# alexlee-gk/video_prediction

Measured on AMD Instinct MI355X. Metric: train frames/sec (whole node), BAIR 64x64 seq30 SAVP, higher is better.
Workload: dtype bf16

## Files before the change

video_prediction_amd/csrc/common.hip:

```cpp
#include <hip/hip_runtime.h>
#include <dlfcn.h>
#include <string.h>
#include "savp_hip.h"
#include "opts.h"
#include "conv_common.h"

extern "C" const char* savp_version(void) { return "savp_hip 0.1 gfx950"; }

thread_local hipEvent_t g_savp_prof_start = nullptr;
thread_local hipEvent_t g_savp_prof_stop = nullptr;

extern "C" int savp_prof_event_create(void** ev) {
    if (!ev) return SAVP_EINVAL;
    hipEvent_t e;
    if (hipEventCreate(&e) != hipSuccess) return SAVP_ELAUNCH;
    *ev = (void*)e;
    return SAVP_OK;
}
extern "C" int savp_prof_event_destroy(void* ev) { return (ev && hipEventDestroy((hipEvent_t)ev) == hipSuccess) ? SAVP_OK : SAVP_EINVAL; }
extern "C" int savp_prof_arm(void* start, void* stop) {
    if ((start == nullptr) != (stop == nullptr)) return SAVP_EINVAL;
    g_savp_prof_start = (hipEvent_t)start; g_savp_prof_stop = (hipEvent_t)stop;
    return SAVP_OK;
}
extern "C" int savp_prof_armed(void) { return g_savp_prof_start != nullptr; }
extern "C" int savp_prof_elapsed_us(void* start, void* stop, float* us) {
    if (!start || !stop || !us) return SAVP_EINVAL;
    float ms = 0.f;
    if (hipEventElapsedTime(&ms, (hipEvent_t)start, (hipEvent_t)stop) != hipSuccess) return SAVP_ELAUNCH;
    *us = ms * 1e3f;
    return SAVP_OK;
}

static struct { const char* name; int value; } g_opts[OPT_COUNT] = {
    {"conv_ring", 0}, {"s2dgrad", 1}, {"thin", 1}, {"wgp_cfg", 0}, {"wgp_split", 0}, {"inorm_min_hw", 64}, {"colsum_2stage", 1},
    {"dense_legacy", 0}, {"cdna_legacy", 0}, {"lstm_fused", 1}, {"ring_dma", 1}, {"lstm_q", 0}, {"ring_wwarm", 1}, {"wgp_dma", 1}, {"ring_early", 1}, {"gate_kernel", 1}, {"gate_alt", 0}, {"gate_cell", 1}, {"gate_wwarm", 1}, {"inorm_fast", 1}, {"inorm_fast_taken", 0}, {"splitk_reduced", 0}, {"ring_fixed", 1}, {"ring_fixed_taken", 0}, {"fd_fixed", 1}, {"fd_fixed_taken", 0},
};
int savp_opt(int id) { return g_opts[id].value; }
void savp_opt_count(int id) { ++g_opts[id].value; }
extern "C" int savp_set_option(const char* name, int value) {
    if (!name) return SAVP_EINVAL;
    for (int i = 0; i < OPT_COUNT; ++i)
        if (!strcmp(g_opts[i].name, name)) { g_opts[i].value = value; return SAVP_OK; }
    return SAVP_EINVAL;
}
extern "C" int savp_get_option(const char* name, int* value) {
    if (!name || !value) return SAVP_EINVAL;
    for (int i = 0; i < OPT_COUNT; ++i)
        if (!strcmp(g_opts[i].name, name)) { *value = g_opts[i].value; return SAVP_OK; }
    return SAVP_EINVAL;
}

typedef int (*rccl_allreduce_fn)(const void*, void*, size_t, int, int, void*, hipStream_t);
extern "C" int savp_allreduce_bucket(void* comm, void* stream, void* buf, int64_t count) {
    if (!comm || !buf || count < 0) return SAVP_EINVAL;
    if (count == 0) return SAVP_OK;
    static rccl_allreduce_fn fn = nullptr;
    if (!fn) {
        void* h = dlopen("librccl.so", RTLD_NOW | RTLD_GLOBAL);
        if (!h) h = dlopen("librccl.so.1", RTLD_NOW | RTLD_GLOBAL);
        if (!h) h = dlopen("/opt/rocm/lib/librccl.so", RTLD_NOW | RTLD_GLOBAL);
        if (!h) return SAVP_ELAUNCH;
        fn = (rccl_allreduce_fn)dlsym(h, "ncclAllReduce");
        if (!fn) return SAVP_ELAUNCH;
    }
    return fn(buf, buf, (size_t)count, 7, 0, comm, (hipStream_t)stream) == 0 ? SAVP_OK : SAVP_ELAUNCH;
}

int splitk_fit(const SavpConvArgs* a, int want, long long block_elems) {
    if (want <= 1) return 1;
    if (!a->ws || a->ws_bytes <= 0 || block_elems <= 0 || (((uintptr_t)a->ws) & 15)) { savp_opt_count(OPT_SPLITK_REDUCED); return 1; }
    const long long fit = a->ws_bytes / (block_elems * (long long)sizeof(float));
    if (fit < want) savp_opt_count(OPT_SPLITK_REDUCED);
    if (fit < 2) return 1;
    return want < fit ? want : (int)fit;
}

__global__ __launch_bounds__(256) void splitk_fold_kernel(float* __restrict__ out, const float* __restrict__ part, int splitk, long long n4, long long n,
                                                          int beta, int Cd, int gap_at, int gap) {
    const long long stride = (long long)gridDim.x * 256;
    for (long long i = (long long)blockIdx.x * 256 + threadIdx.x; i < n4; i += stride) {
        float4 s = beta ? reinterpret_cast<const float4*>(out)[i] : make_float4(0.f, 0.f, 0.f, 0.f);
        for (int k = 0; k < splitk; ++k) {
            const float4 v = reinterpret_cast<const float4*>(part + (long long)k * n)[i];
            s.x += v.x; s.y += v.y; s.z += v.z; s.w += v.w;
        }
        if (gap) {
            const int c = (int)((i * 4) % Cd);
            float* e = &s.x;
#pragma unroll
            for (int j = 0; j < 4; ++j)
                if (c + j >= gap_at && c + j < gap_at + gap) e[j] = beta ? reinterpret_cast<const float*>(out)[i * 4 + j] : 0.f;
        }
        reinterpret_cast<float4*>(out)[i] = s;
    }
}

__global__ __launch_bounds__(256) void splitk_fold_scalar_kernel(float* __restrict__ out, const float* __restrict__ part, int splitk, long long n, int beta,
                                                                 int Cd, int gap_at, int gap) {
    const long long stride = (long long)gridDim.x * 256;
    for (long long i = (long long)blockIdx.x * 256 + threadIdx.x; i < n; i += stride) {
        const int c = (int)(i % Cd);
        if (gap && c >= gap_at && c < gap_at + gap) { if (!beta) out[i] = 0.f; continue; }
        float s = beta ? out[i] : 0.f;
        for (int k = 0; k < splitk; ++k) s += part[(long long)k * n + i];
        out[i] = s;
    }
}

void splitk_fold(float* out, const float* part, int splitk, long long n, int beta, int Cd, int gap_at, int gap, hipStream_t st) {
    const bool vec = (n % 4 == 0) && (Cd % 4 == 0) && ((((uintptr_t)out) & 15) == 0) && ((((uintptr_t)part) & 15) == 0);
    const long long work = vec ? n / 4 : n;
    long long blocks = (work + 255) / 256;
    if (blocks > 2048) blocks = 2048;
    if (blocks < 1) blocks = 1;
    if (vec) hipLaunchKernelGGL(splitk_fold_kernel, dim3((unsigned)blocks), dim3(256), 0, st, out, part, splitk, n / 4, n, beta, Cd, gap_at, gap);
    else hipLaunchKernelGGL(splitk_fold_scalar_kernel, dim3((unsigned)blocks), dim3(256), 0, st, out, part, splitk, n, beta, Cd, gap_at, gap);
}

typedef float fold_f4 __attribute__((ext_vector_type(4)));
template <bool VEC>
__global__ __launch_bounds__(256) void wgrad_fold_kernel(float* __restrict__ out, const float* __restrict__ part, int nsplit, long long n, long long slice) {
    const long long i = (long long)blockIdx.x * 256 + threadIdx.x;
    if (i >= n) return;
    if constexpr (VEC) {
        fold_f4 s = reinterpret_cast<const fold_f4*>(out)[i];
        const fold_f4* __restrict__ q = reinterpret_cast<const fold_f4*>(part) + i;
        const long long st4 = slice >> 2;
        int k = 0;
        for (; k + 8 <= nsplit; k += 8) {
            fold_f4 v[8];
#pragma unroll
            for (int j = 0; j < 8; ++j) v[j] = __builtin_nontemporal_load(q + (long long)(k + j) * st4);
#pragma unroll
            for (int j = 0; j < 8; ++j) s += v[j];
        }
        for (; k < nsplit; ++k) s += __builtin_nontemporal_load(q + (long long)k * st4);
        reinterpret_cast<fold_f4*>(out)[i] = s;
    } else {
        float s = out[i];
        for (int k = 0; k < nsplit; ++k) s += part[(long long)k * slice + i];
        out[i] = s;
    }
}

void wgrad_fold(float* out, const float* part, int nsplit, long long n, hipStream_t st, long long slice) {
    if (nsplit < 1 || n <= 0) return;
    if (slice <= 0) slice = n;
    const bool vec = (n % 4 == 0) && (slice % 4 == 0) && ((((uintptr_t)out) & 15) == 0) && ((((uintptr_t)part) & 15) == 0);
    const long long work = vec ? n / 4 : n;
    const unsigned blocks = (unsigned)((work + 255) / 256);
    if (vec) hipLaunchKernelGGL(wgrad_fold_kernel<true>, dim3(blocks), dim3(256), 0, st, out, part, nsplit, work, slice);
    else hipLaunchKernelGGL(wgrad_fold_kernel<false>, dim3(blocks), dim3(256), 0, st, out, part, nsplit, work, slice);
}
```

video_prediction_amd/csrc/conv_gate.hip:

```cpp
#include "conv_common.h"
#include "opts.h"
#include <hip/hip_ext.h>
#include <type_traits>

extern thread_local hipEvent_t g_savp_prof_start;
extern thread_local hipEvent_t g_savp_prof_stop;

struct GateP {
    const unsigned short* x;
    const uint4* wfrag;
    unsigned short* y;
    double* stats;
    const void* zero16;
    int N, Cy, mtiles, ntiles;
    int wwarm;
    int F; float eps, forget_bias;
    const float* c_prev; long long cp_sn, cp_sp;
    const float *g1, *b1, *g2, *b2;
    float* c_new;
    int nh; void* h[4]; long long h_sn[4], h_sp[4]; int h16;
    float *mean1, *rstd1, *mean2, *rstd2;
};

__device__ __attribute__((aligned(16))) unsigned g_gate_zero[4] = {0u, 0u, 0u, 0u};

#ifdef SAVP_GATE_STAMPS
__device__ unsigned long long g_gate_t[4][8];
__constant__ int g_gate_blk = 0;
#define GT(i) do { if ((int)blockIdx.x == g_gate_blk && (threadIdx.x & 63) == 0) g_gate_t[threadIdx.x >> 6][i] = __builtin_readcyclecounter(); } while (0)
extern "C" int savp_debug_gate_times(unsigned long long* out) { return hipMemcpyFromSymbol(out, HIP_SYMBOL(g_gate_t), sizeof(g_gate_t)) == hipSuccess ? 0 : -1; }
extern "C" int savp_debug_gate_block(int b) { return hipMemcpyToSymbol(HIP_SYMBOL(g_gate_blk), &b, sizeof(int)) == hipSuccess ? 0 : -1; }
#else
#define GT(i) do {} while (0)
#endif

__device__ __forceinline__ void gate_touch4(const void* gsrc, unsigned lds_dst) {
    unsigned keep;
    asm volatile("s_mov_b32 %0, m0\n\ts_mov_b32 m0, %2\n\ts_nop 0\n\tglobal_load_lds_dword %1, off\n\ts_mov_b32 m0, %0"
                 : "=&s"(keep) : "v"(gsrc), "s"(lds_dst) : "memory");
}

__device__ __forceinline__ void gate_dma16(const void* gsrc, unsigned lds_dst) {
    unsigned keep;
    asm volatile("s_mov_b32 %0, m0\n\ts_mov_b32 m0, %2\n\ts_nop 0\n\tglobal_load_lds_dwordx4 %1, off\n\ts_mov_b32 m0, %0"
                 : "=&s"(keep) : "v"(gsrc), "s"(lds_dst) : "memory");
}

template <int S, int CIN, int TM, int TN, int NWN>
struct GateCfg {
    static constexpr int KH = 5, KW = 5, PAD = 2, TAPS = KH * KW;
    static constexpr int KSPLIT = 4 / NWN;
    static constexpr int PIX = 32 * TM;
    static constexpr int C8 = CIN / 8;
    static constexpr int C8P = (C8 & 1) ? C8 : C8 + 1;
    static constexpr int PXB = C8P * 16;
    static constexpr int TC = S >= 16 ? 16 : 8;
    static constexpr int TR = (S * S >= PIX) ? PIX / TC : S;
    static constexpr int NI = PIX / (TR * TC);
    static constexpr int PR = TR + 2 * PAD, PC = TC + 2 * PAD;
    static constexpr int RPAD = (256 - (4 * PXB) % 256) % 256;
    static constexpr int RP = PC * PXB + RPAD;
    static constexpr int IMGB = PR * RP;
    static constexpr int PATCHB = NI * IMGB;
    static constexpr int NCH = TAPS * C8;
    static constexpr int KS = (NCH + 1) / 2;
    static constexpr int KPAD = 8;
    static constexpr int ETABB = ((2 * (KS + KPAD) * 4) + 15) & ~15;
    static constexpr int NCW = 32 * TN;
    static constexpr int NC = NCW * NWN;
    static constexpr int TILEB = 32 * 32 * 4;
    static constexpr int XB = (KSPLIT > 1 ? TM / 2 : 0) * TN * TILEB;
    static constexpr int TP = NC / 2 + 4;
    static constexpr int STGB = PIX * TP * 4;
    static constexpr int STATB = KSPLIT * NC * 2 * 4;
    static constexpr int EPIB = (4 * XB > STGB ? 4 * XB : STGB) + STATB;
    static constexpr int WARMB = 256;
    static constexpr int LDSB = (PATCHB + ETABB + WARMB) > EPIB ? (PATCHB + ETABB + WARMB) : EPIB;
    static constexpr int TPI = NI == 1 ? (S / TR) * (S / TC) : 1;
    static constexpr int PPR = PC * C8P;
    static constexpr int NJ = (PPR + 63) / 64;
    static constexpr int aoff(int i) { return ((i * 32) / (TR * TC)) * IMGB + (((i * 32) % (TR * TC)) / TC) * RP; }
    static_assert(CIN % 8 == 0 && S % TC == 0 && S % TR == 0 && (TM == 4 || TM == 8) && (TN == 1 || TN == 2) && (NWN == 1 || NWN == 2) && TR * TC * NI == PIX && 32 % TC == 0, "shape");
    static_assert(LDSB <= 160 * 1024, "LDS");
};

template <int TM, int TN, int I>
__device__ __forceinline__ void gate_sched() {
    constexpr int M = TM * TN, ND = TM + 1, NV = TN;
    if constexpr (I < M) {
        constexpr int d = (ND * (I + 1)) / M - (ND * I) / M;
        constexpr int v = (NV * (I + 1)) / M - (NV * I) / M;
        if constexpr (d > 0) __builtin_amdgcn_sched_group_barrier(0x100, d, 0);
        if constexpr (v > 0) __builtin_amdgcn_sched_group_barrier(0x020, v, 0);
        __builtin_amdgcn_sched_group_barrier(0x008, 1, 0);
        gate_sched<TM, TN, I + 1>();
    }
}

template <int S, int CIN, int TM, int TN, int NWN, bool CELL = false>
__global__ __launch_bounds__(256, (2 * GateCfg<S, CIN, TM, TN, NWN>::LDSB <= 160 * 1024 ? 2 : 1)) void conv_gate_kernel(GateP p) {
    GT(0);
    using G = GateCfg<S, CIN, TM, TN, NWN>;
    constexpr int KS = G::KS, NC = G::NC;
    extern __shared__ __attribute__((aligned(16))) unsigned char gsm[];
    unsigned char* patch = gsm;
    unsigned* etab = reinterpret_cast<unsigned*>(gsm + G::PATCHB);
    const int tid = threadIdx.x, lane = tid & 63;
    const int wave = __builtin_amdgcn_readfirstlane(tid >> 6);
    const int nw = wave % NWN, kq = wave / NWN;
    constexpr int KSPLIT = G::KSPLIT;
    const int l31 = lane & 31, khalf = lane >> 5;

    const int logical = xcd_logical((int)blockIdx.x, p.mtiles * p.ntiles);
    const int nt = logical / p.mtiles, mt = logical - nt * p.mtiles;
    const int n0 = nt * NC;
    int img0, ty0, tx0;
    if constexpr (G::NI == 1) {
        img0 = mt / G::TPI;
        const int tr = mt % G::TPI;
        ty0 = (tr / (S / G::TC)) * G::TR; tx0 = (tr % (S / G::TC)) * G::TC;
    } else {
        img0 = mt * G::NI; ty0 = 0; tx0 = 0;
    }

    if (p.wwarm) {
        const int nwg = p.mtiles * p.ntiles, qx = nwg >> 3, rx = nwg & 7, xcd = (int)blockIdx.x & 7;
        const int first = xcd < rx ? xcd * (qx + 1) : rx * (qx + 1) + (xcd - rx) * qx;
        const int cnt = qx + (xcd < rx ? 1 : 0);
        const int l_lo = max(first, nt * p.mtiles), l_hi = min(first + cnt, (nt + 1) * p.mtiles);
        const int share = max(l_hi - l_lo, 1), mine = min(max(logical - l_lo, 0), share - 1);
        constexpr int BLK = TN * NWN * KS * 1024;
        const int chunk = ((BLK + share - 1) / share + 8191) & ~8191;
        const unsigned char* wb = reinterpret_cast<const unsigned char*>(p.wfrag) + (size_t)(n0 / 32) * KS * 1024;
        const unsigned warm_lds = (unsigned)(uintptr_t)(gsm + G::PATCHB + G::ETABB);
        for (int off = wave * 8192; off < chunk && mine * chunk + off < BLK; off += 4 * 8192) {
            const int a = min(mine * chunk + off + lane * 128, BLK - 4);
            gate_touch4(wb + a, warm_lds);
        }
    }
    {
        const unsigned patch_lds = (unsigned)(uintptr_t)patch;
        const unsigned char* xb = reinterpret_cast<const unsigned char*>(p.x);
        const unsigned long long zero16 = (unsigned long long)(uintptr_t)p.zero16;
        int rel[G::NJ];
#pragma unroll
        for (int j = 0; j < G::NJ; ++j) {
            const int piece = j * 64 + lane;
            const int px = piece / G::C8P, ch = piece - px * G::C8P;
            const int ix = tx0 + px - G::PAD;
            const bool ok = piece < G::PPR && ch < G::C8 && (unsigned)ix < (unsigned)S;
            rel[j] = ok ? (ix * CIN + ch * 8) * 2 : -1;
        }
        for (int row = wave; row < G::NI * G::PR; row += 4) {
            const int im = row / G::PR, py = row - im * G::PR;
            const int n = img0 + im, iy = ty0 + py - G::PAD;
            const bool row_ok = (unsigned)iy < (unsigned)S && n < p.N;
            const unsigned char* rb = xb + ((long long)n * S + iy) * (long long)(S * CIN * 2);
            const unsigned lds_row = patch_lds + (unsigned)(im * G::IMGB + py * G::RP);
            if (!row_ok) {
#pragma unroll
                for (int j = 0; j < G::NJ; ++j)
                    if (j * 64 + lane < G::PPR) *reinterpret_cast<uint4*>(patch + im * G::IMGB + py * G::RP + (j * 64 + lane) * 16) = make_uint4(0u, 0u, 0u, 0u);
                continue;
            }
#pragma unroll
            for (int j = 0; j < G::NJ; ++j) {
                if (j * 64 + lane < G::PPR) {
                    const unsigned long long g = (row_ok && rel[j] >= 0) ? (unsigned long long)(uintptr_t)(rb + rel[j]) : zero16;
                    gate_dma16(reinterpret_cast<const void*>((uintptr_t)g), lds_row + (unsigned)(j * 1024));
                }
            }
        }
    }
    GT(1);
    for (int c = tid; c < 2 * (KS + G::KPAD); c += 256) {
        const int cc = c < G::NCH ? c : 0;
        const int tap = cc / G::C8, ch = cc - tap * G::C8;
        etab[c] = (unsigned)((tap / G::KW) * G::RP + (tap % G::KW) * G::PXB + ch * 16);
    }

    constexpr int KSW = (KS + KSPLIT - 1) / KSPLIT;
    const int ks0 = kq * KSW, ks1 = min(KS, ks0 + KSW);
    const uint4* __restrict__ bsrc[TN];
#pragma unroll
    for (int j = 0; j < TN; ++j) bsrc[j] = p.wfrag + ((long long)(n0 / 32 + nw * TN + j) * KS) * 64 + lane;
    constexpr int PF = (TM * TN >= 8) ? 4 : 8;
#ifndef SAVP_GATE_ABL
#define SAVP_GATE_ABL 0
#endif
    uint4 bq[PF][TN];
#pragma unroll
    for (int u = 0; u < PF; ++u)
#pragma unroll
        for (int j = 0; j < TN; ++j) bq[u][j] = bsrc[j][(long long)(ks0 + u) * 64];

    const unsigned a0 = (unsigned)((l31 / G::TC) * G::RP + (l31 % G::TC) * G::PXB);
    f32x16 acc[TM][TN];
#pragma unroll
    for (int i = 0; i < TM; ++i)
#pragma unroll
        for (int j = 0; j < TN; ++j)
#pragma unroll
            for (int r = 0; r < 16; ++r) acc[i][j][r] = 0.f;

    GT(2);
    asm volatile("s_waitcnt vmcnt(0)" ::: "memory");
    __syncthreads();
    GT(3);

    bf16x8 af[2][TM];
    auto load_a = [&](bf16x8 (&dst)[TM], unsigned off) {
        const unsigned char* a = patch + a0 + off;
#pragma unroll
        for (int i = 0; i < TM; ++i) dst[i] = *reinterpret_cast<const bf16x8*>(a + G::aoff(i));
    };
    const unsigned* etl = etab + khalf;
    load_a(af[0], etl[2 * ks0]);
    unsigned off_next = etl[2 * (ks0 + 1)];
    auto kstep = [&](int k, auto uc, auto steadyc) {
        constexpr int u = decltype(uc)::value;
        constexpr bool STEADY = decltype(steadyc)::value;
        if (!(SAVP_GATE_ABL & 2)) {
            load_a(af[(u + 1) & 1], off_next);
            off_next = etl[2 * (k + 2)];
        }
        bf16x8 bf[TN];
#pragma unroll
        for (int j = 0; j < TN; ++j) bf[j] = __builtin_bit_cast(bf16x8, bq[u % PF][j]);
#pragma unroll
        for (int i = 0; i < TM; ++i)
#pragma unroll
            for (int j = 0; j < TN; ++j) {
                if (!(SAVP_GATE_ABL & 4)) acc[i][j] = __builtin_amdgcn_mfma_f32_32x32x16_bf16(af[u & 1][i], bf[j], acc[i][j], 0, 0, 0);
                else asm volatile("" :: "v"(af[u & 1][i]), "v"(bf[j]));
            }
        if (!(SAVP_GATE_ABL & 1)) {
#pragma unroll
            for (int j = 0; j < TN; ++j) bq[u % PF][j] = bsrc[j][(long long)(k + PF) * 64];
        }
        if constexpr (STEADY) gate_sched<TM, TN, 0>();
    };
    using U0 = std::integral_constant<int, 0>; using U1 = std::integral_constant<int, 1>;
    using U2 = std::integral_constant<int, 2>; using U3 = std::integral_constant<int, 3>;
    using U4 = std::integral_constant<int, 4>; using U5 = std::integral_constant<int, 5>;
    using U6 = std::integral_constant<int, 6>; using U7 = std::integral_constant<int, 7>;
    static_assert(PF == 4 || PF == 8, "the loop is unrolled PF k-steps: the B ring's slots are compile-time registers");
    int k = ks0;
    auto body = [&](auto... us) { (kstep(k + decltype(us)::value, us, std::true_type{}), ...); };
    auto tail = [&](auto... us) { ((k < ks1 ? (kstep(k, us, std::false_type{}), ++k, 0) : 0), ...); };
    if constexpr (PF == 4) {
        for (; k + 4 <= ks1; k += 4) body(U0{}, U1{}, U2{}, U3{});
        tail(U0{}, U1{}, U2{});
    } else {
        for (; k + 8 <= ks1; k += 8) body(U0{}, U1{}, U2{}, U3{}, U4{}, U5{}, U6{}, U7{});
        tail(U0{}, U1{}, U2{}, U3{}, U4{}, U5{}, U6{});
    }
    GT(4);

    __syncthreads();
    constexpr int TMH = TM / 2, TMQ = TM / 4;
    float4* xbuf = reinterpret_cast<float4*>(gsm);
    auto xput = [&](int wslot, auto ilo_c, auto ni_c) {
        constexpr int ILO = decltype(ilo_c)::value, NI_ = decltype(ni_c)::value;
        float4* dst = xbuf + (size_t)wslot * (G::XB / 16) + lane;
#pragma unroll
        for (int i = ILO; i < ILO + NI_; ++i)
#pragma unroll
            for (int j = 0; j < TN; ++j)
#pragma unroll
                for (int g = 0; g < 4; ++g) {
                    dst[(((i - ILO) * TN + j) * 4 + g) * 64] = make_float4(acc[i][j][4 * g], acc[i][j][4 * g + 1], acc[i][j][4 * g + 2], acc[i][j][4 * g + 3]);
                    if (g == 3) __builtin_amdgcn_sched_barrier(0);
                }
    };
    auto xadd = [&](int wslot, auto ilo_c, auto ni_c) {
        constexpr int ILO = decltype(ilo_c)::value, NI_ = decltype(ni_c)::value;
        const float4* src = xbuf + (size_t)wslot * (G::XB / 16) + lane;
#pragma unroll
        for (int i = ILO; i < ILO + NI_; ++i)
#pragma unroll
            for (int j = 0; j < TN; ++j)
#pragma unroll
                for (int g = 0; g < 4; ++g) {
                    const float4 v = src[(((i - ILO) * TN + j) * 4 + g) * 64];
                    acc[i][j][4 * g] += v.x; acc[i][j][4 * g + 1] += v.y; acc[i][j][4 * g + 2] += v.z; acc[i][j][4 * g + 3] += v.w;
                    if (g == 3) __builtin_amdgcn_sched_barrier(0);
                }
    };
    using IC0 = std::integral_constant<int, 0>; using ICH = std::integral_constant<int, TMH>; using ICQ = std::integral_constant<int, TMQ>;
    using ICHQ = std::integral_constant<int, TMH + TMQ>;
    const int odd = kq & 1, hi = kq >> 1;
    if (!odd) xput(wave, ICH{}, ICH{}); else xput(wave, IC0{}, ICH{});
    __syncthreads();
    if (!odd) xadd(wave ^ NWN, IC0{}, ICH{}); else xadd(wave ^ NWN, ICH{}, ICH{});
    __syncthreads();
    if constexpr (KSPLIT == 4) {
        if (!odd && !hi) xput(wave, ICQ{}, ICQ{});
        else if (!odd && hi) xput(wave, IC0{}, ICQ{});
        else if (odd && !hi) xput(wave, ICHQ{}, ICQ{});
        else xput(wave, ICH{}, ICQ{});
        __syncthreads();
        if (!odd && !hi) xadd(wave ^ 2, IC0{}, ICQ{});
        else if (!odd && hi) xadd(wave ^ 2, ICQ{}, ICQ{});
        else if (odd && !hi) xadd(wave ^ 2, ICH{}, ICQ{});
        else xadd(wave ^ 2, ICHQ{}, ICQ{});
        __syncthreads();
    }
    GT(5);

#ifndef SAVP_CELL_ABL
#define SAVP_CELL_ABL 0
#endif
    if constexpr (CELL) {
        static_assert(TN == 1 && NWN == 1 && G::TR == S && G::TC == S, "plane-local cell: whole images per tile, one 32-column block per workgroup");
        constexpr int TMFc = TM / 4, HWI = S * S;
        constexpr int FINS[4] = {0, TMQ, TMH, TMH + TMQ};
        const int fin = kq == 0 ? 0 : (kq == 2 ? TMQ : (kq == 1 ? TMH : TMH + TMQ));
        const int F = p.F;
        const int ch = l31 >> 2, g = l31 & 3;
        const int cch = nt * 8 + ch;
        const int pc = g * F + cch;
        float* stat = reinterpret_cast<float*>(gsm + G::PIX * 32 * 2);
        float* stat2 = stat + 4 * 32 * 2;
        unsigned short* T16 = reinterpret_cast<unsigned short*>(gsm);
        float v[TMFc][16];
        auto grab = [&](auto fin_c) {
            constexpr int FIN = decltype(fin_c)::value;
#pragma unroll
            for (int i = 0; i < TMFc; ++i)
#pragma unroll
                for (int r = 0; r < 16; ++r) v[i][r] = acc[FIN + i][0][r];
        };
        if (kq == 0) grab(IC0{}); else if (kq == 2) grab(ICQ{}); else if (kq == 1) grab(ICH{}); else grab(ICHQ{});
        (void)FINS;
        const int pix0 = fin * 32 + 4 * khalf;
        const int im = pix0 / HWI;
        const int n = img0 + im;
        const bool live = n < p.N;
        const int nn = live ? n : p.N - 1;
        constexpr int NE = TMFc * 4;
        auto erow = [&](int i, int m) { return pix0 + i * 32 + g + 8 * m; };
        float cp[NE];
        if (p.c_prev) {
            const float* __restrict__ cpb = p.c_prev + (long long)nn * p.cp_sn + cch;
#pragma unroll
            for (int i = 0; i < TMFc; ++i)
#pragma unroll
// ... 127 lines not shown
            const int pix = idx >> 2, gg = idx & 3;
            const int imp = pix / HWI, px = pix - imp * HWI;
            const int np = img0 + imp;
            if (np >= p.N) continue;
            const uint4 w = *reinterpret_cast<const uint4*>(T16 + pix * 32 + gg * 8);
            *reinterpret_cast<uint4*>(p.y + ((long long)np * HWI + px) * (long long)p.Cy + gg * F + nt * 8) = w;
        }
        GT(7);
        return;
    }

    float* stat = reinterpret_cast<float*>(gsm + (4 * G::XB > G::STGB ? 4 * G::XB : G::STGB));
    unsigned* T = reinterpret_cast<unsigned*>(gsm);
    constexpr int TMF = TM / KSPLIT;
    auto finish = [&](auto fin_c) {
        constexpr int FIN = decltype(fin_c)::value;
        const bool oddl = lane & 1;
#pragma unroll
        for (int i = FIN; i < FIN + TMF; ++i)
#pragma unroll
            for (int j = 0; j < TN; ++j) {
                const int cp = (nw * G::NCW + 32 * j + (l31 & ~1)) >> 1;
#pragma unroll
                for (int m = 0; m < 8; ++m) {
                    const float e = acc[i][j][2 * m], o = acc[i][j][2 * m + 1];
                    const float en = __builtin_bit_cast(float, __builtin_amdgcn_mov_dpp(__builtin_bit_cast(int, e), 0xB1, 0xF, 0xF, true));
                    const float on = __builtin_bit_cast(float, __builtin_amdgcn_mov_dpp(__builtin_bit_cast(int, o), 0xB1, 0xF, 0xF, true));
                    const int r = 2 * m + (oddl ? 1 : 0);
                    const int row = i * 32 + (r & 3) + 8 * (r >> 2) + 4 * khalf;
                    typedef __bf16 bf16x2 __attribute__((ext_vector_type(2)));
                    T[row * G::TP + cp] = oddl ? __builtin_bit_cast(unsigned, bf16x2{(__bf16)on, (__bf16)o}) : __builtin_bit_cast(unsigned, bf16x2{(__bf16)e, (__bf16)en});
                }
            }
        if (p.stats) {
#pragma unroll
            for (int j = 0; j < TN; ++j) {
                float sm = 0.f, q = 0.f;
#pragma unroll
                for (int i = FIN; i < FIN + TMF; ++i)
#pragma unroll
                    for (int r = 0; r < 16; ++r) { const float v = acc[i][j][r]; sm += v; q += v * v; }
                sm += __shfl_xor(sm, 32); q += __shfl_xor(q, 32);
                if (khalf == 0) { stat[(kq * NC + nw * G::NCW + 32 * j + l31) * 2] = sm; stat[(kq * NC + nw * G::NCW + 32 * j + l31) * 2 + 1] = q; }
            }
        }
    };
    if constexpr (KSPLIT == 4) {
        if (!odd && !hi) finish(IC0{});
        else if (!odd && hi) finish(ICQ{});
        else if (odd && !hi) finish(ICH{});
        else finish(ICHQ{});
    } else {
        if (!odd) finish(IC0{}); else finish(ICH{});
    }
    __syncthreads();
    GT(6);
    {
        constexpr int CH = NC / 8;
        for (int idx = tid; idx < G::PIX * CH; idx += 256) {
            const int pix = idx / CH, c8 = idx - pix * CH;
            const int im = pix / (G::TR * G::TC), rr = pix - im * (G::TR * G::TC);
            const int n = img0 + im;
            if (n >= p.N) continue;
            const int oy = ty0 + rr / G::TC, ox = tx0 + rr % G::TC;
            const uint4 v = *reinterpret_cast<const uint4*>(T + pix * G::TP + c8 * 4);
            unsigned short* dst = p.y + (((long long)n * S + oy) * S + ox) * (long long)p.Cy + n0 + c8 * 8;
            *reinterpret_cast<uint4*>(dst) = v;
        }
    }
    if (p.stats) {
        constexpr int WPI = KSPLIT / G::NI;
        for (int i = tid; i < G::NI * NC * 2; i += 256) {
            const int im = i / (NC * 2), rem = i - im * (NC * 2);
            const int n = img0 + im;
            if (n >= p.N) continue;
            float t = 0.f;
#pragma unroll
            for (int o = 0; o < WPI; ++o) {
                const int ord = im * WPI + o;
                const int q_ = KSPLIT == 4 ? (((ord & 1) << 1) | (ord >> 1)) : ord;
                t += stat[q_ * NC * 2 + rem];
            }
            unsafeAtomicAdd(p.stats + ((long long)n * p.Cy + n0 + (rem >> 1)) * 2 + (rem & 1), (double)t);
        }
    }
    GT(7);
}

#define GATE_PACK_PAD_KSTEPS 8
__global__ __launch_bounds__(256) void pack_gate_weights_kernel(const float* __restrict__ src, int taps, int Cx, int Cy, uint4* __restrict__ out, int il_F) {
    const int C8 = Cx >> 3, nch = taps * C8, KS = (nch + 1) >> 1;
    const long long total = (long long)(Cy >> 5) * KS * 64;
    for (long long t = total + (long long)blockIdx.x * 256 + threadIdx.x; t < total + GATE_PACK_PAD_KSTEPS * 64; t += (long long)gridDim.x * 256)
        out[t] = make_uint4(0u, 0u, 0u, 0u);
    for (long long t = (long long)blockIdx.x * 256 + threadIdx.x; t < total; t += (long long)gridDim.x * 256) {
        const int lane = (int)(t & 63);
        const long long r = t >> 6;
        const int ks = (int)(r % KS), cb = (int)(r / KS);
        const int c = 2 * ks + (lane >> 5);
        typedef __bf16 bf16x2 __attribute__((ext_vector_type(2)));
        unsigned w[4] = {0u, 0u, 0u, 0u};
        if (c < nch) {
            const int tap = c / C8, ch = c - tap * C8;
            const int l = lane & 31, col = il_F ? (l & 3) * il_F + cb * 8 + (l >> 2) : cb * 32 + l;
            const float* s = src + ((long long)tap * Cx + ch * 8) * Cy + col;
#pragma unroll
            for (int j = 0; j < 4; ++j) w[j] = __builtin_bit_cast(unsigned, bf16x2{(__bf16)s[(long long)(2 * j) * Cy], (__bf16)s[(long long)(2 * j + 1) * Cy]});
        }
        out[t] = make_uint4(w[0], w[1], w[2], w[3]);
    }
}

extern "C" int64_t savp_gate_weights_bytes(int32_t taps, int32_t Cx, int32_t Cy) {
    if (taps < 1 || Cx < 8 || (Cx & 7) || Cy < 32 || (Cy & 31)) return 0;
    const long long KS = ((long long)taps * (Cx >> 3) + 1) >> 1;
    return ((long long)(Cy >> 5) * KS + GATE_PACK_PAD_KSTEPS) * 64 * 16;
}

extern "C" int savp_pack_gate_weights(void* stream, const float* src, int32_t taps, int32_t Cx, int32_t Cy, void* out, int32_t interleave) {
    if (!src || !out || !savp_gate_weights_bytes(taps, Cx, Cy) || (((uintptr_t)out) & 15)) return SAVP_EINVAL;
    if (interleave && (Cy % 4 != 0 || (Cy / 4) % 8 != 0)) return SAVP_EINVAL;
    const long long total = savp_gate_weights_bytes(taps, Cx, Cy) / 16 - GATE_PACK_PAD_KSTEPS * 64;
    unsigned nb = (unsigned)((total + 255) / 256);
    if (nb > 4096) nb = 4096;
    hipLaunchKernelGGL(pack_gate_weights_kernel, dim3(nb), dim3(256), 0, (hipStream_t)stream, src, taps, Cx, Cy, (uint4*)out, interleave ? Cy / 4 : 0);
    return hipGetLastError() == hipSuccess ? SAVP_OK : SAVP_ELAUNCH;
}

template <int S, int CIN, int TM, int TN, int NWN, bool CELL = false>
static hipError_t launch_gate(const GateP& p, hipStream_t st) {
    using G = GateCfg<S, CIN, TM, TN, NWN>;
    static bool attr = false;
    if (!attr) {
        hipFuncSetAttribute((const void*)conv_gate_kernel<S, CIN, TM, TN, NWN, CELL>, hipFuncAttributeMaxDynamicSharedMemorySize, G::LDSB);
        attr = true;
    }
    const dim3 grid((unsigned)(p.mtiles * p.ntiles));
    if (g_savp_prof_start) {
        hipExtLaunchKernelGGL((conv_gate_kernel<S, CIN, TM, TN, NWN, CELL>), grid, dim3(256), G::LDSB, st, g_savp_prof_start, g_savp_prof_stop, 0, p);
        g_savp_prof_start = g_savp_prof_stop = nullptr;
    } else {
        hipLaunchKernelGGL((conv_gate_kernel<S, CIN, TM, TN, NWN, CELL>), grid, dim3(256), G::LDSB, st, p);
    }
    return hipGetLastError();
}

#define GATE_SHAPES(X)                                                                                                    \
    X(32, 72, 8, 1, 2, 0) X(16, 136, 4, 1, 1, 0) X(8, 264, 4, 1, 1, 0)        \
    X(32, 96, 8, 1, 2, 0) X(16, 160, 4, 1, 1, 0)                            \
    X(32, 64, 8, 1, 2, 0) X(16, 128, 4, 1, 1, 0) X(8, 256, 4, 1, 1, 0)      \
    X(32, 136, 8, 1, 2, 0) X(32, 264, 4, 1, 2, 0) X(16, 264, 4, 1, 2, 0)    \
    X(32, 72, 4, 1, 2, 1) X(16, 136, 4, 1, 2, 2) X(32, 96, 4, 1, 2, 1) X(16, 160, 4, 1, 2, 2) X(32, 72, 4, 1, 1, 4) X(32, 72, 4, 2, 1, 8)

static bool gate_shape_ok(const SavpConvArgs* a) {
#define X(S_, C_, TM_, TN_, NWN_, ALT_) if (a->H == S_ && a->Cx == C_) return true;
    GATE_SHAPES(X)
#undef X
    return false;
}

bool conv_gate_applies(const SavpConvArgs* a) {
    if (!savp_opt(OPT_GATE_KERNEL)) return false;
    if (!(a->mode == SAVP_CONV_FPROP && a->precision == SAVP_PREC_BF16 && a->src_bf16 && a->out_bf16 && a->w_frag && !a->bias && !a->aux &&
          a->act == SAVP_ACT_NONE && !a->beta && !a->dst_gap && !a->nb_ws && a->splitk <= 1))
        return false;
    if (!(a->D == 1 && a->Do == 1 && a->kd == 1 && a->kh == 5 && a->kw == 5 && a->sd == 1 && a->sh == 1 && a->sw == 1 && a->pd == 0 && a->ph == 2 &&
          a->pw == 2 && a->H == a->W && a->Ho == a->H && a->Wo == a->W))
        return false;
    if (!(a->x_sw == a->Cx && a->x_sh == (long long)a->W * a->Cx && a->x_sn == (long long)a->H * a->W * a->Cx && a->y_sw == a->Cy &&
          a->y_sh == (long long)a->W * a->Cy && a->y_sn == (long long)a->H * a->W * a->Cy && aligned16(a->x) && aligned16(a->y) && aligned16(a->w_frag)))
        return false;
    if ((a->Cy & 127) || a->N < 1 || (a->stats && (((uintptr_t)a->stats) & 7))) return false;
    return gate_shape_ok(a);
}

bool conv_gate_try(const SavpConvArgs* a, hipStream_t st, int* rc) {
    if (!conv_gate_applies(a)) return false;
    static const void* zero_of[64] = {nullptr};
    int dev_ord = 0;
    if (hipGetDevice(&dev_ord) != hipSuccess || dev_ord < 0 || dev_ord >= 64) dev_ord = 0;
    if (!zero_of[dev_ord] && hipGetSymbolAddress((void**)&zero_of[dev_ord], HIP_SYMBOL(g_gate_zero)) != hipSuccess) { *rc = SAVP_ELAUNCH; return true; }
    GateP p;
    p.x = (const unsigned short*)a->x; p.wfrag = (const uint4*)a->w_frag; p.y = (unsigned short*)a->y; p.stats = (double*)a->stats;
    p.zero16 = zero_of[dev_ord]; p.N = a->N; p.Cy = a->Cy; p.wwarm = savp_opt(OPT_GATE_WWARM);
    hipError_t err = hipErrorInvalidValue;
    const int alt = savp_opt(OPT_GATE_ALT);
    bool done = false;
#define X(S_, C_, TM_, TN_, NWN_, ALT_)                                                                  \
    if (!done && a->H == S_ && a->Cx == C_ && (want ? (ALT_ & want) != 0 : ALT_ == 0)) {                 \
        using G = GateCfg<S_, C_, TM_, TN_, NWN_>;                                                       \
        p.mtiles = G::NI == 1 ? a->N * G::TPI : (a->N + G::NI - 1) / G::NI; p.ntiles = a->Cy / G::NC;    \
        err = launch_gate<S_, C_, TM_, TN_, NWN_>(p, st);                                                \
        done = true;                                                                                     \
    }
    { const int want = alt; GATE_SHAPES(X) }
    { const int want = 0; GATE_SHAPES(X) }
#undef X
    *rc = err == hipSuccess ? SAVP_OK : SAVP_ELAUNCH;
    return true;
}

#define GATE_CELL_SHAPES(X) X(16, 136, 8) X(8, 264, 4) X(16, 160, 8) X(16, 128, 8) X(8, 256, 4)

bool conv_gate_cell_try(const SavpConvLstmCellArgs* c, hipStream_t st, int* rc) {
    const SavpConvArgs* a = &c->conv;
    const SavpLstmArgs* g = &c->gates;
    if (!savp_opt(OPT_GATE_KERNEL) || !savp_opt(OPT_GATE_CELL) || !a->w_frag_il) return false;
    SavpConvArgs b = *a;
    b.w_frag = a->w_frag_il;
    if (!b.stats) b.stats = (double*)(uintptr_t)16;
    if (!conv_gate_applies(&b)) return false;
    bool shape = false;
#define X(S_, C_, TM_) if (a->H == S_ && a->Cx == C_) shape = true;
    GATE_CELL_SHAPES(X)
#undef X
    if (!shape) return false;
    if (g->no_norm || !g->gates_bf16 || g->F * 4 != a->Cy || g->N != a->N || g->HW != a->H * a->W || g->nh < 0 || g->nh > 4 || !g->gamma1 || !g->beta1 ||
        !g->gamma2 || !g->beta2 || !g->c_new || !g->mean1 || !g->rstd1 || !g->mean2 || !g->rstd2 || (g->F & 7))
        return false;
    if (g->c_prev.sp * (long long)g->HW >= (1ll << 31)) return false;
    for (int i = 0; i < g->nh; ++i)
        if (g->h[i].sp * (long long)g->HW >= (1ll << 31)) return false;
    static const void* zero_of[64] = {nullptr};
    int dev_ord = 0;
    if (hipGetDevice(&dev_ord) != hipSuccess || dev_ord < 0 || dev_ord >= 64) dev_ord = 0;
    if (!zero_of[dev_ord] && hipGetSymbolAddress((void**)&zero_of[dev_ord], HIP_SYMBOL(g_gate_zero)) != hipSuccess) { *rc = SAVP_ELAUNCH; return true; }
    GateP p;
    p.x = (const unsigned short*)a->x; p.wfrag = (const uint4*)a->w_frag_il; p.y = (unsigned short*)a->y; p.stats = nullptr;
    p.zero16 = zero_of[dev_ord]; p.N = a->N; p.Cy = a->Cy; p.wwarm = savp_opt(OPT_GATE_WWARM);
    p.F = g->F; p.eps = g->eps; p.forget_bias = g->forget_bias;
    p.c_prev = (const float*)g->c_prev.p; p.cp_sn = g->c_prev.sn; p.cp_sp = g->c_prev.sp;
    p.g1 = g->gamma1; p.b1 = g->beta1; p.g2 = g->gamma2; p.b2 = g->beta2;
    p.c_new = g->c_new; p.nh = g->nh; p.h16 = g->h_bf16;
    for (int i = 0; i < 4; ++i) { p.h[i] = i < g->nh ? g->h[i].p : nullptr; p.h_sn[i] = i < g->nh ? g->h[i].sn : 0; p.h_sp[i] = i < g->nh ? g->h[i].sp : 0; }
    p.mean1 = g->mean1; p.rstd1 = g->rstd1; p.mean2 = g->mean2; p.rstd2 = g->rstd2;
    hipError_t err = hipErrorInvalidValue;
#define X(S_, C_, TM_)                                                                                   \
    if (a->H == S_ && a->Cx == C_) {                                                                     \
        using G = GateCfg<S_, C_, TM_, 1, 1>;                                                            \
        p.mtiles = (a->N + G::NI - 1) / G::NI; p.ntiles = a->Cy / 32;                                    \
        err = launch_gate<S_, C_, TM_, 1, 1, true>(p, st);                                               \
    }
    GATE_CELL_SHAPES(X)
#undef X
    *rc = err == hipSuccess ? SAVP_OK : SAVP_ELAUNCH;
    return true;
}
```

video_prediction_amd/csrc/opts.h:

```cpp
#pragma once

enum SavpOptId {
    OPT_CONV_RING = 0,
    OPT_S2DGRAD,
    OPT_THIN,
    OPT_WGP_CFG,
    OPT_WGP_SPLIT,
    OPT_INORM_MIN_HW,
    OPT_COLSUM_2STAGE,
    OPT_DENSE_LEGACY,
    OPT_CDNA_LEGACY,
    OPT_LSTM_FUSED,
    OPT_RING_DMA,
    OPT_LSTM_Q,
    OPT_RING_WWARM,
    OPT_WGP_DMA,
    OPT_RING_EARLY,
    OPT_GATE_KERNEL,
    OPT_GATE_ALT,
    OPT_GATE_CELL,
    OPT_GATE_WWARM,
    OPT_INORM_FAST,
    OPT_INORM_FAST_TAKEN,
    OPT_SPLITK_REDUCED,
    OPT_RING_FIXED,
    OPT_RING_FIXED_TAKEN,
    OPT_FD_FIXED,
    OPT_FD_FIXED_TAKEN,
    OPT_COUNT
};

int savp_opt(int id);
void savp_opt_count(int id);

#ifdef __HIPCC__
template <int BYTES>
__device__ __forceinline__ void kernarg_warm() {
    constexpr int LINES = (BYTES + 63) / 64;
    const unsigned long long ka = (unsigned long long)__builtin_amdgcn_kernarg_segment_ptr();
    unsigned t[LINES];
#pragma unroll
    for (int i = 0; i < LINES; ++i) asm volatile("s_load_dword %0, %1, %2" : "=&s"(t[i]) : "s"(ka), "n"(i * 64) : "memory");
    asm volatile("s_waitcnt lgkmcnt(0)" ::: "memory");
#pragma unroll
    for (int i = 0; i < LINES; ++i) asm volatile("" :: "s"(t[i]));
}
#endif
```

video_prediction_amd/lib.py:

```python
import ctypes
import os

import torch

from . import debug as _debug

_HERE = os.path.dirname(os.path.abspath(__file__))
LIB_PATH = os.environ.get('SAVP_LIB') or os.path.join(_HERE, 'libsavp_hip.so')

c_i32, c_i64, c_f32, c_vp = ctypes.c_int32, ctypes.c_int64, ctypes.c_float, ctypes.c_void_p

CONV_FPROP, CONV_DGRAD, CONV_WGRAD = 0, 1, 2
ACT_NONE, ACT_LRELU, ACT_SIGMOID, ACT_DLRELU_FROM_OUT = 0, 1, 2, 3


class SavpConvArgs(ctypes.Structure):
    _fields_ = [
        ('mode', c_i32),
        ('N', c_i32), ('D', c_i32), ('H', c_i32), ('W', c_i32), ('Cx', c_i32),
        ('Do', c_i32), ('Ho', c_i32), ('Wo', c_i32), ('Cy', c_i32),
        ('kd', c_i32), ('kh', c_i32), ('kw', c_i32),
        ('sd', c_i32), ('sh', c_i32), ('sw', c_i32),
        ('pd', c_i32), ('ph', c_i32), ('pw', c_i32),
        ('beta', c_i32), ('act', c_i32), ('alpha', c_f32), ('splitk', c_i32), ('tile', c_i32), ('precision', c_i32),
        ('x', c_vp), ('x_sn', c_i64), ('x_sd', c_i64), ('x_sh', c_i64), ('x_sw', c_i64),
        ('y', c_vp), ('y_sn', c_i64), ('y_sd', c_i64), ('y_sh', c_i64), ('y_sw', c_i64),
        ('w', c_vp), ('bias', c_vp), ('aux', c_vp), ('w_bf16', c_vp),
        ('src_bf16', c_i32), ('out_bf16', c_i32), ('stats', c_vp),
        ('ws', c_vp), ('ws_bytes', c_i64),
        ('dst_gap_at', c_i32), ('dst_gap', c_i32),
        ('nb_x', c_vp), ('nb_x_sn', c_i64), ('nb_x_sp', c_i64), ('nb_mean', c_vp), ('nb_rstd', c_vp), ('nb_gamma', c_vp), ('nb_beta', c_vp),
        ('nb_ws', c_vp), ('nb_c0', c_i32), ('nb_nc', c_i32), ('nb_act', c_i32), ('nb_alpha', c_f32),
        ('w_frag', c_vp), ('w_frag_il', c_vp),
    ]


class SavpJpegArgs(ctypes.Structure):
    _fields_ = [
        ('N', c_i32), ('width', c_i32), ('height', c_i32), ('components', c_i32),
        ('h', c_i32 * 3), ('v', c_i32 * 3), ('blocks_w', c_i32 * 3), ('blocks_h', c_i32 * 3), ('block_offset', c_i32 * 3),
        ('total_blocks', c_i32), ('out_h', c_i32), ('out_w', c_i32),
        ('coef', c_vp), ('qtab', c_vp), ('window', c_vp), ('out', c_vp), ('ws', c_vp), ('ws_bytes', c_i64),
    ]


_lib = None


def get():
    global _lib
    if _lib is None:
        if not os.path.exists(LIB_PATH):
            raise RuntimeError(
                'libsavp_hip.so not found at %s -- build it first (python -c "import __graft_entry__ as g; g.build()"). '
                'video_prediction_amd has no non-HIP fallback.' % LIB_PATH)
        lib = ctypes.CDLL(LIB_PATH)
        lib.savp_version.restype = ctypes.c_char_p
        _declare(lib)
        _lib = lib
        _forward_env_options(lib)
    if _debug.POISON['lds']:
        return _LdsPoisonProxy(_lib)
    return _lib


def get_raw():
    lib = get()
    return lib._lib if isinstance(lib, _LdsPoisonProxy) else lib


class _LdsPoisonProxy(object):

    def __init__(self, lib):
        self._lib = lib

    def __getattr__(self, name):
        fn = getattr(self._lib, name)
        at = getattr(fn, 'argtypes', None)
        if not name.startswith('savp_') or name.startswith(('savp_debug_', 'savp_prof_')) or not at or at[0] is not c_vp or \
                name in ('savp_allreduce_bucket',):
            return fn
        poison = self._lib.savp_debug_poison_lds

        def call(st, *args):
            poison(st, _debug.NAN_WORD, None)
            _debug.COUNTS['lds'] += 1
            return fn(st, *args)
        return call


OPTION_NAMES = ('conv_ring', 's2dgrad', 'thin', 'wgp_cfg', 'wgp_split', 'inorm_min_hw', 'colsum_2stage', 'dense_legacy', 'cdna_legacy',
                'lstm_fused', 'ring_dma', 'lstm_q', 'ring_wwarm', 'wgp_dma', 'ring_early', 'gate_kernel', 'gate_alt', 'gate_cell', 'gate_wwarm', 'inorm_fast', 'inorm_fast_taken', 'splitk_reduced', 'ring_fixed', 'ring_fixed_taken', 'fd_fixed', 'fd_fixed_taken')


def set_option(name, value):
    check(get().savp_set_option(name.encode(), int(value)), 'savp_set_option(%s)' % name)


def get_option(name):
    v = c_i32()
    check(get().savp_get_option(name.encode(), ctypes.byref(v)), 'savp_get_option(%s)' % name)
    return v.value


def _forward_env_options(lib):
    for name in OPTION_NAMES:
        v = os.environ.get('SAVP_' + name.upper())
        if v is not None:
            check(lib.savp_set_option(name.encode(), int(v)), 'savp_set_option(%s)' % name)


EXPORTS = {}


def _sig(lib, name, argtypes, restype=c_i32):
    try:
        fn = getattr(lib, name)
    except AttributeError:
        if os.environ.get('SAVP_LIB'):
            return None
        raise
    fn.argtypes = argtypes
    fn.restype = restype
    EXPORTS[name] = fn
    return fn


def _declare(lib):
    P = ctypes.POINTER
    _sig(lib, 'savp_conv', [c_vp, P(SavpConvArgs)])
    _sig(lib, 'savp_conv_workspace_bytes', [P(SavpConvArgs)], restype=c_i64)
    _sig(lib, 'savp_conv_special', [P(SavpConvArgs)])
    _sig(lib, 'savp_gate_weights_bytes', [c_i32, c_i32, c_i32], restype=c_i64)
    _sig(lib, 'savp_conv_stats_ok', [P(SavpConvArgs)])
    _sig(lib, 'savp_fd_fixed_count', [])
    _sig(lib, 'savp_fd_fixed_probe', [c_i32, c_i32, P(c_i64), c_i32])
    _sig(lib, 'savp_set_option', [ctypes.c_char_p, c_i32])
    _sig(lib, 'savp_get_option', [ctypes.c_char_p, P(c_i32)])
    _sig(lib, 'savp_allreduce_bucket', [c_vp, c_vp, c_vp, c_i64])
    _sig(lib, 'savp_tiled_z_weff', [c_vp, c_vp, c_i32, c_i32, c_i32, c_i32, c_i32, c_i32, c_i32, c_i32, c_vp])
    _sig(lib, 'savp_tiled_z_grad', [c_vp, c_vp, c_i32, c_i64, c_i32, c_i32, c_i32, c_vp, c_i32, c_vp, c_i32, c_vp, c_i64])
    _sig(lib, 'savp_tiled_z_workspace_bytes', [c_i64, c_i32], restype=c_i64)
    _sig(lib, 'savp_eval_fold_ws_floats', [c_i32, c_i32, c_i32, c_i32], restype=c_i64)
    _sig(lib, 'savp_jpeg_workspace_bytes', [P(SavpJpegArgs)], restype=c_i64)
    _sig(lib, 'savp_convgru_large_chunk', [c_i32, c_i32])
    _sig(lib, 'savp_convgru_large_ws_bytes', [c_i32, c_i32, c_i32], restype=c_i64)
    _sig(lib, 'savp_convgru_ln_chunk', [c_i32, c_i32])
    _sig(lib, 'savp_convgru_ln_ws_bytes', [c_i32, c_i32, c_i32], restype=c_i64)
    _sig(lib, 'savp_arena_health_chunk', [])
    _sig(lib, 'savp_arena_health_ws_bytes', [c_i64], restype=c_i64)
    for name, argtypes in _EXTRA_SIGS.items():
        _sig(lib, name, argtypes)


_EXTRA_SIGS = {}


def register(name, argtypes):
    _EXTRA_SIGS[name] = argtypes
    if _lib is not None:
        _sig(_lib, name, argtypes)


def source_id():
    import hashlib
    h = hashlib.sha256()
    root = os.path.dirname(_HERE)
    files = []
    for d, pat in ((os.path.join(_HERE, 'csrc'), ('.hip', '.h')), (os.path.join(root, 'include'), ('.h',)), (_HERE, ('.json',))):
        for f in sorted(os.listdir(d)):
            if f.endswith(pat) and (d != _HERE or f.startswith('tuning_gfx950_')):
                files.append(os.path.join(d, f))
    for f in files:
        h.update(os.path.basename(f).encode())
        with open(f, 'rb') as fh:
            h.update(fh.read())
    return h.hexdigest()[:16]


def stream():
    return ctypes.c_void_p(torch.cuda.current_stream().cuda_stream)


def check(rc, what):
    if rc != 0:
        raise RuntimeError('%s failed with code %d' % (what, rc))


def ptr(t):
    return ctypes.c_void_p(t.data_ptr()) if t is not None else ctypes.c_void_p(0)


def require_device(*tensors):
    for t in tensors:
        if t is None:
            continue
        if not t.is_cuda:
            raise RuntimeError('video_prediction_amd kernels need device tensors (got %s); there is no CPU path' % t.device)
        if t.dtype != torch.float32:
            raise RuntimeError('expected float32, got %s' % t.dtype)


def require_stats(*tensors):
    for t in tensors:
        if t is None:
            continue
        if not t.is_cuda:
            raise RuntimeError('video_prediction_amd kernels need device tensors (got %s); there is no CPU path' % t.device)
        if t.dtype != torch.float64 or (t.data_ptr() & 7):
            raise RuntimeError('statistics workspaces are float64 (kernels.stats_ws), got %s' % t.dtype)


def require_device_any(*tensors):
    for t in tensors:
        if t is None:
            continue
        if not t.is_cuda:
            raise RuntimeError('video_prediction_amd kernels need device tensors (got %s); there is no CPU path' % t.device)
        if t.dtype not in (torch.float32, torch.bfloat16):
            raise RuntimeError('expected float32 or bfloat16, got %s' % t.dtype)


class SavpView(ctypes.Structure):
    _fields_ = [('p', c_vp), ('sn', c_i64), ('sp', c_i64)]


class SavpInormArgs(ctypes.Structure):
    _fields_ = [
        ('N', c_i32), ('HW', c_i32), ('C', c_i32), ('act', c_i32), ('alpha', c_f32), ('eps', c_f32),
        ('x', SavpView), ('gamma', c_vp), ('beta', c_vp),
        ('nout', c_i32), ('out', SavpView * 4), ('mean', c_vp), ('rstd', c_vp),
        ('ndy', c_i32), ('dy', SavpView * 4), ('dx', SavpView), ('dx_beta', c_i32),
        ('dgamma', c_vp), ('dbeta', c_vp), ('ws', c_vp), ('ws_clean', c_i32),
        ('out_c0', c_i32 * 4), ('out_nc', c_i32 * 4), ('dy_c0', c_i32 * 4), ('dy_nc', c_i32 * 4), ('out_bf16', c_i32),
        ('stats_ready', c_i32), ('stats_shift', c_vp), ('dx_bf16', c_i32),
    ]


class SavpGnormArgs(ctypes.Structure):
    _fields_ = [('norm', SavpInormArgs), ('G', c_i32), ('ws_group', c_vp), ('dsum', c_vp)]


class SavpPlainActArgs(ctypes.Structure):
    _fields_ = [
        ('N', c_i32), ('HW', c_i32), ('C', c_i32), ('act', c_i32), ('alpha', c_f32), ('x', SavpView), ('add', c_vp),
# ... 280 lines not shown
```

Baseline: 11320.

## Add 2D XCD tile grouping and early weight prefetch to gate conv kernel

Result: no change. 11390 (median of 6 runs) (+0.6%).

```diff
diff --git a/video_prediction_amd/csrc/common.hip b/video_prediction_amd/csrc/common.hip
--- a/video_prediction_amd/csrc/common.hip
+++ b/video_prediction_amd/csrc/common.hip
@@ -34,7 +34,7 @@
 
 static struct { const char* name; int value; } g_opts[OPT_COUNT] = {
     {"conv_ring", 0}, {"s2dgrad", 1}, {"thin", 1}, {"wgp_cfg", 0}, {"wgp_split", 0}, {"inorm_min_hw", 64}, {"colsum_2stage", 1},
-    {"dense_legacy", 0}, {"cdna_legacy", 0}, {"lstm_fused", 1}, {"ring_dma", 1}, {"lstm_q", 0}, {"ring_wwarm", 1}, {"wgp_dma", 1}, {"ring_early", 1}, {"gate_kernel", 1}, {"gate_alt", 0}, {"gate_cell", 1}, {"gate_wwarm", 1}, {"inorm_fast", 1}, {"inorm_fast_taken", 0}, {"splitk_reduced", 0}, {"ring_fixed", 1}, {"ring_fixed_taken", 0}, {"fd_fixed", 1}, {"fd_fixed_taken", 0},
+    {"dense_legacy", 0}, {"cdna_legacy", 0}, {"lstm_fused", 1}, {"ring_dma", 1}, {"lstm_q", 0}, {"ring_wwarm", 1}, {"wgp_dma", 1}, {"ring_early", 1}, {"gate_kernel", 1}, {"gate_alt", 0}, {"gate_cell", 1}, {"gate_wwarm", 1}, {"inorm_fast", 1}, {"inorm_fast_taken", 0}, {"splitk_reduced", 0}, {"ring_fixed", 1}, {"ring_fixed_taken", 0}, {"fd_fixed", 1}, {"fd_fixed_taken", 0}, {"gate_early", 1}, {"gate_xcd2d", 1},
 };
 int savp_opt(int id) { return g_opts[id].value; }
 void savp_opt_count(int id) { ++g_opts[id].value; }
diff --git a/video_prediction_amd/csrc/conv_gate.hip b/video_prediction_amd/csrc/conv_gate.hip
--- a/video_prediction_amd/csrc/conv_gate.hip
+++ b/video_prediction_amd/csrc/conv_gate.hip
@@ -13,7 +13,7 @@
     double* stats;
     const void* zero16;
     int N, Cy, mtiles, ntiles;
-    int wwarm;
+    int sw;
     int F; float eps, forget_bias;
     const float* c_prev; long long cp_sn, cp_sp;
     const float *g1, *b1, *g2, *b2;
@@ -111,8 +111,25 @@
     constexpr int KSPLIT = G::KSPLIT;
     const int l31 = lane & 31, khalf = lane >> 5;
 
-    const int logical = xcd_logical((int)blockIdx.x, p.mtiles * p.ntiles);
-    const int nt = logical / p.mtiles, mt = logical - nt * p.mtiles;
+    const int nwg = p.mtiles * p.ntiles;
+    const int logical = xcd_logical((int)blockIdx.x, nwg);
+    int nt, mt, run_lo, run_n;
+    const int xig = p.sw >> 8;
+    if (xig == 1) {
+        nt = logical / p.mtiles; mt = logical - nt * p.mtiles;
+        run_lo = nt * p.mtiles; run_n = p.mtiles;
+    } else {
+        const int sh = 31 - __builtin_clz(xig);
+        const int qm = p.mtiles >> sh, rm = p.mtiles - (qm << sh);
+        const int big = rm * (qm + 1) * p.ntiles;
+        const bool in_big = logical < big;
+        const int cnt = in_big ? qm + 1 : qm, l2 = in_big ? logical : logical - big;
+        const int gi = l2 / (cnt * p.ntiles), lr = l2 - gi * cnt * p.ntiles;
+        nt = lr / cnt;
+        const int mr = lr - nt * cnt;
+        mt = (in_big ? gi * cnt : rm * (qm + 1) + gi * cnt) + mr;
+        run_lo = logical - mr; run_n = cnt;
+    }
     const int n0 = nt * NC;
     int img0, ty0, tx0;
     if constexpr (G::NI == 1) {
@@ -123,11 +140,26 @@
         img0 = mt * G::NI; ty0 = 0; tx0 = 0;
     }
 
-    if (p.wwarm) {
-        const int nwg = p.mtiles * p.ntiles, qx = nwg >> 3, rx = nwg & 7, xcd = (int)blockIdx.x & 7;
+    constexpr int KSW = (KS + KSPLIT - 1) / KSPLIT;
+    const int ks0 = kq * KSW, ks1 = min(KS, ks0 + KSW);
+    const uint4* __restrict__ bsrc[TN];
+#pragma unroll
+    for (int j = 0; j < TN; ++j) bsrc[j] = p.wfrag + ((long long)(n0 / 32 + nw * TN + j) * KS) * 64 + lane;
+    constexpr int PF = (TM * TN >= 8) ? 4 : 8;
+    uint4 bq[PF][TN];
+    auto b_first = [&]() {
+#pragma unroll
+        for (int u = 0; u < PF; ++u)
+#pragma unroll
+            for (int j = 0; j < TN; ++j) bq[u][j] = bsrc[j][(long long)(ks0 + u) * 64];
+    };
+    if (p.sw & 2) b_first();
+
+    if (p.sw & 1) {
+        const int qx = nwg >> 3, rx = nwg & 7, xcd = (int)blockIdx.x & 7;
         const int first = xcd < rx ? xcd * (qx + 1) : rx * (qx + 1) + (xcd - rx) * qx;
         const int cnt = qx + (xcd < rx ? 1 : 0);
-        const int l_lo = max(first, nt * p.mtiles), l_hi = min(first + cnt, (nt + 1) * p.mtiles);
+        const int l_lo = max(first, run_lo), l_hi = min(first + cnt, run_lo + run_n);
         const int share = max(l_hi - l_lo, 1), mine = min(max(logical - l_lo, 0), share - 1);
         constexpr int BLK = TN * NWN * KS * 1024;
         const int chunk = ((BLK + share - 1) / share + 8191) & ~8191;
@@ -179,20 +211,10 @@
         etab[c] = (unsigned)((tap / G::KW) * G::RP + (tap % G::KW) * G::PXB + ch * 16);
     }
 
-    constexpr int KSW = (KS + KSPLIT - 1) / KSPLIT;
-    const int ks0 = kq * KSW, ks1 = min(KS, ks0 + KSW);
-    const uint4* __restrict__ bsrc[TN];
-#pragma unroll
-    for (int j = 0; j < TN; ++j) bsrc[j] = p.wfrag + ((long long)(n0 / 32 + nw * TN + j) * KS) * 64 + lane;
-    constexpr int PF = (TM * TN >= 8) ? 4 : 8;
 #ifndef SAVP_GATE_ABL
 #define SAVP_GATE_ABL 0
 #endif
-    uint4 bq[PF][TN];
-#pragma unroll
-    for (int u = 0; u < PF; ++u)
-#pragma unroll
-        for (int j = 0; j < TN; ++j) bq[u][j] = bsrc[j][(long long)(ks0 + u) * 64];
+    if (!(p.sw & 2)) b_first();
 
     const unsigned a0 = (unsigned)((l31 / G::TC) * G::RP + (l31 % G::TC) * G::PXB);
     f32x16 acc[TM][TN];
@@ -626,6 +648,19 @@
     X(32, 136, 8, 1, 2, 0) X(32, 264, 4, 1, 2, 0) X(16, 264, 4, 1, 2, 0)    \
     X(32, 72, 4, 1, 2, 1) X(16, 136, 4, 1, 2, 2) X(32, 96, 4, 1, 2, 1) X(16, 160, 4, 1, 2, 2) X(32, 72, 4, 1, 1, 4) X(32, 72, 4, 2, 1, 8)
 
+static int gate_xig(const SavpConvArgs* a, int mtiles, int ntiles) {
+    const int opt = savp_opt(OPT_GATE_XCD2D);
+    int best = 1;
+    long long best_cost = 0;
+    for (int g = 1; g <= 8 && g <= mtiles && opt > 0; g *= 2) {
+        if (opt > 1) { if (g <= opt) best = g; continue; }
+        const long long in_x = 8 / g < ntiles ? 8 / g : ntiles, w_x = g > 8 / ntiles ? g : 8 / ntiles;
+        const long long cost = in_x * a->N * a->H * a->W + w_x * 25 * a->Cy;
+        if (g == 1 || cost < best_cost) { best = g; best_cost = cost; }
+    }
+    return best;
+}
+
 static bool gate_shape_ok(const SavpConvArgs* a) {
 #define X(S_, C_, TM_, TN_, NWN_, ALT_) if (a->H == S_ && a->Cx == C_) return true;
     GATE_SHAPES(X)
@@ -656,7 +691,7 @@
     if (!zero_of[dev_ord] && hipGetSymbolAddress((void**)&zero_of[dev_ord], HIP_SYMBOL(g_gate_zero)) != hipSuccess) { *rc = SAVP_ELAUNCH; return true; }
     GateP p;
     p.x = (const unsigned short*)a->x; p.wfrag = (const uint4*)a->w_frag; p.y = (unsigned short*)a->y; p.stats = (double*)a->stats;
-    p.zero16 = zero_of[dev_ord]; p.N = a->N; p.Cy = a->Cy; p.wwarm = savp_opt(OPT_GATE_WWARM);
+    p.zero16 = zero_of[dev_ord]; p.N = a->N; p.Cy = a->Cy; p.sw = (savp_opt(OPT_GATE_WWARM) ? 1 : 0) | (savp_opt(OPT_GATE_EARLY) ? 2 : 0);
     hipError_t err = hipErrorInvalidValue;
     const int alt = savp_opt(OPT_GATE_ALT);
     bool done = false;
@@ -664,6 +699,7 @@
     if (!done && a->H == S_ && a->Cx == C_ && (want ? (ALT_ & want) != 0 : ALT_ == 0)) {                 \
         using G = GateCfg<S_, C_, TM_, TN_, NWN_>;                                                       \
         p.mtiles = G::NI == 1 ? a->N * G::TPI : (a->N + G::NI - 1) / G::NI; p.ntiles = a->Cy / G::NC;    \
+        p.sw = (p.sw & 255) | gate_xig(a, p.mtiles, p.ntiles) << 8;                                      \
         err = launch_gate<S_, C_, TM_, TN_, NWN_>(p, st);                                                \
         done = true;                                                                                     \
     }
@@ -701,7 +737,7 @@
     if (!zero_of[dev_ord] && hipGetSymbolAddress((void**)&zero_of[dev_ord], HIP_SYMBOL(g_gate_zero)) != hipSuccess) { *rc = SAVP_ELAUNCH; return true; }
     GateP p;
     p.x = (const unsigned short*)a->x; p.wfrag = (const uint4*)a->w_frag_il; p.y = (unsigned short*)a->y; p.stats = nullptr;
-    p.zero16 = zero_of[dev_ord]; p.N = a->N; p.Cy = a->Cy; p.wwarm = savp_opt(OPT_GATE_WWARM);
+    p.zero16 = zero_of[dev_ord]; p.N = a->N; p.Cy = a->Cy; p.sw = (savp_opt(OPT_GATE_WWARM) ? 1 : 0) | (savp_opt(OPT_GATE_EARLY) ? 2 : 0);
     p.F = g->F; p.eps = g->eps; p.forget_bias = g->forget_bias;
     p.c_prev = (const float*)g->c_prev.p; p.cp_sn = g->c_prev.sn; p.cp_sp = g->c_prev.sp;
     p.g1 = g->gamma1; p.b1 = g->beta1; p.g2 = g->gamma2; p.b2 = g->beta2;
@@ -713,6 +749,7 @@
     if (a->H == S_ && a->Cx == C_) {                                                                     \
         using G = GateCfg<S_, C_, TM_, 1, 1>;                                                            \
         p.mtiles = (a->N + G::NI - 1) / G::NI; p.ntiles = a->Cy / 32;                                    \
+        p.sw = (p.sw & 255) | gate_xig(a, p.mtiles, p.ntiles) << 8;                                      \
         err = launch_gate<S_, C_, TM_, 1, 1, true>(p, st);                                               \
     }
     GATE_CELL_SHAPES(X)
diff --git a/video_prediction_amd/csrc/opts.h b/video_prediction_amd/csrc/opts.h
--- a/video_prediction_amd/csrc/opts.h
+++ b/video_prediction_amd/csrc/opts.h
@@ -27,6 +27,8 @@
     OPT_RING_FIXED_TAKEN,
     OPT_FD_FIXED,
     OPT_FD_FIXED_TAKEN,
+    OPT_GATE_EARLY,
+    OPT_GATE_XCD2D,
     OPT_COUNT
 };
 
diff --git a/video_prediction_amd/lib.py b/video_prediction_amd/lib.py
--- a/video_prediction_amd/lib.py
+++ b/video_prediction_amd/lib.py
@@ -90,7 +90,7 @@
 
 
 OPTION_NAMES = ('conv_ring', 's2dgrad', 'thin', 'wgp_cfg', 'wgp_split', 'inorm_min_hw', 'colsum_2stage', 'dense_legacy', 'cdna_legacy',
-                'lstm_fused', 'ring_dma', 'lstm_q', 'ring_wwarm', 'wgp_dma', 'ring_early', 'gate_kernel', 'gate_alt', 'gate_cell', 'gate_wwarm', 'inorm_fast', 'inorm_fast_taken', 'splitk_reduced', 'ring_fixed', 'ring_fixed_taken', 'fd_fixed', 'fd_fixed_taken')
+                'lstm_fused', 'ring_dma', 'lstm_q', 'ring_wwarm', 'wgp_dma', 'ring_early', 'gate_kernel', 'gate_alt', 'gate_cell', 'gate_wwarm', 'inorm_fast', 'inorm_fast_taken', 'splitk_reduced', 'ring_fixed', 'ring_fixed_taken', 'fd_fixed', 'fd_fixed_taken', 'gate_early', 'gate_xcd2d')
 
 
 def set_option(name, value):
```
